# inferflow/inferflow

Hardware: AMD Instinct MI355X
Metric: decode tokens/sec, Llama-2-7B Q4 batch=1 greedy (whole job) (higher is better)
Workload: dtype i8 (Q8 activations x Q4_B32T1A weights, i32 dot, f32 scale, f16 I/O); 1 GPU; llama2_7b decode, Q4_B32T1A weights + F16 lm_head, F16 KV cache, batch 1 greedy, 16-token prompt, context 21..1851; parallelism=single, weights_bytes=4309647360

## Files before the change

inferflow_amd/csrc/ifa_decode_attn.h:

```cpp
#pragma once
#include "ifa_decode_kernels.h"
#include "ifa_decode_route.h"

namespace ifa {

struct DecAttnParams {
    const half_t *q;
    const half_t *k_new;
    const half_t *v_new;
    uint8_t *kcache, *vcache;
    const int *state;
    const float *rope_tab;
    int heads, kv_heads, kv_q8;
    float kq_scale;
    int rope_order, rope_cols;
    int alibi, alibi_base, alibi_total;
    half_t *out;
    int max_ctx;
    int8_t *xq;
    long long *trace;
    const void *batch_rows;
    int q_stride;
    int skip_store;
};
// ... 61 lines not shown
    int pos;
    unsigned *err;
    long long timeout_ticks;
    unsigned long long *att_gran;
};

__host__ __device__ inline int att_gran_count(int heads, int hd) { return heads * hd / 4 + 2 * (heads * hd / 32) + heads; }

template <int HD, bool Q8, int PB, bool KT>
struct DecAttnRegs {
    static constexpr int DG = HD / 8, NSPLIT = 256 / DG, VPRE = PB / NSPLIT;
    static constexpr int KBYTES = (HD / 32) * 34;
    static constexpr int KALIGN = HD == 128 ? 8 : (HD == 64 ? 4 : 2);
    uint32_t kreg[Q8 ? 1 : HD / 2];
    uint32_t kq32[(Q8 && KALIGN >= 4) ? KBYTES / 4 : 1];
    uint16_t kq16[(Q8 && KALIGN < 4) ? KBYTES / 2 : 1];
    u32x4 kt[KT ? PB / NSPLIT : 1];
    u32x4 vreg[Q8 ? 1 : VPRE];
    uint32_t vqs[Q8 ? VPRE : 1], vqc[Q8 ? VPRE : 1][2];
    float rope_cs, rope_sn;
    half_t q_in, k_in, v_in;
};

template <int HD, bool Q8, bool BATCH, int PB, bool KT, bool FUSED, int PHASE = 0>
__device__ __forceinline__ void dec_attn_body(char *smem, const half_t *pq, const uint8_t *pkc, const uint8_t *pvc, int pheads, int pkvh,
                                              const DecAttnParams &P, const int h_in, const DecAttnFusedIn &F, DecAttnRegs<HD, Q8, PB, KT> &R)
{
    int pos_b = 0;
    if constexpr (FUSED) pos_b = F.pos;
    if constexpr (BATCH) {
        const DecAttnBatchRow br = reinterpret_cast<const DecAttnBatchRow *>(P.batch_rows)[blockIdx.y];
        pkc = br.kc; pvc = br.vc; pos_b = br.n_ctx - 1;
        pq += (size_t)blockIdx.y * P.q_stride;
    }
#define IFA_GP(T, p) ((const __attribute__((address_space(1))) T *)(p))
    uint8_t *const kcw = BATCH ? const_cast<uint8_t *>(pkc) : P.kcache;
    uint8_t *const vcw = BATCH ? const_cast<uint8_t *>(pvc) : P.vcache;
    const float *const rope_tab = BATCH ? P.rope_tab + (size_t)blockIdx.y * HD : P.rope_tab;
    half_t *const outp = BATCH ? P.out + (size_t)blockIdx.y * pheads * HD : P.out;
    static_assert(HD % 8 == 0 && HD <= 128 && (!Q8 || HD % 32 == 0), "head size: multiples of 8 up to 128 (Q8 rows: whole 32-blocks)");
    constexpr int DG = HD / 8;
    constexpr int NSPLIT = 256 / DG;
    half_t *qs = reinterpret_cast<half_t *>(smem);
    half_t *kn = qs + HD;
    half_t *vn = kn + HD;
    float *red = reinterpret_cast<float *>(vn + HD);
    float *opart = red + 16;
    static_assert(!KT || (!Q8 && !BATCH && (DG & (DG - 1)) == 0 && PB % NSPLIT == 0), "K tile through LDS: F16 rows, one query, power-of-two pieces per row");
    static_assert(!(FUSED && BATCH), "the fused tail is a single-query kernel");
    static_assert(PB >= NSPLIT && PB <= DEC_ATTN_MIN_ROWS, "prefetch bucket");
    uint8_t *ktile = reinterpret_cast<uint8_t *>(opart + NSPLIT * HD);
    half_t *S = reinterpret_cast<half_t *>(ktile + (KT ? (size_t)PB * HD * 2 : 0));
    const int h = h_in, tid = threadIdx.x, lane = tid & 63, wave = tid >> 6;
    const int group = pheads / pkvh;
    const int kvh = h / group;
    bool writer = (h % group) == 0;
    if constexpr (BATCH) writer = writer && !P.skip_store;
    const int kv_dim = pkvh * HD;
    const size_t row_bytes = Q8 ? (size_t)(kv_dim / 32) * 34 : (size_t)kv_dim * 2;
    const size_t head_off = Q8 ? (size_t)((kvh * HD) / 32) * 34 : (size_t)kvh * HD * 2;

    constexpr int KBYTES = (HD / 32) * 34;
    constexpr int KALIGN = HD == 128 ? 8 : (HD == 64 ? 4 : 2);
    auto &kreg = R.kreg; auto &kq32 = R.kq32; auto &kq16 = R.kq16; auto &kt = R.kt; auto &vreg = R.vreg; auto &vqs = R.vqs; auto &vqc = R.vqc;
    float &rope_cs = R.rope_cs, &rope_sn = R.rope_sn;
    half_t &q_in = R.q_in, &k_in = R.k_in, &v_in = R.v_in;
    auto load_k = [&](int j) {
        const uint8_t *rowp = pkc + (size_t)j * row_bytes + head_off;
        if constexpr (Q8) {
            if constexpr (KALIGN == 8) {
#pragma unroll
                for (int i = 0; i < KBYTES / 8; i++) {
// ... 48 lines not shown
        const int j = min(sp + NSPLIT * i, BATCH ? pos_b : (FUSED ? min(pos_b, PB - 1) : PB - 1));
        if constexpr (!Q8) {
            vreg[i] = IFA_GP(u32x4, pvc + (size_t)j * row_bytes + head_off)[dg];
        } else {
            const auto *blk = IFA_GP(uint16_t, pvc + (size_t)j * row_bytes + vq_off);
            typedef uint32_t u32x2_a2 __attribute__((ext_vector_type(2), aligned(2)));
            vqs[i] = blk[0];
            const u32x2_a2 cw = *IFA_GP(u32x2_a2, blk + 1 + (dg % 4) * 4);
            vqc[i][0] = cw[0]; vqc[i][1] = cw[1];
        }
    }
    }
    if constexpr (PHASE == 1) return;

    const bool tr = P.trace != nullptr && tid == 0;
    if (tr) P.trace[h * 8 + 0] = wall_clock64();
    const int pos = (BATCH || FUSED) ? pos_b : *(const __attribute__((address_space(4))) int *)(P.state + 1);
    const int n_ctx = pos + 1;
    if constexpr (FUSED) {
        if (tid < HD) {
            const unsigned long long *gq = F.gran + (size_t)h * HD + tid, *gk = F.gran + (size_t)(pheads + kvh) * HD + tid,
                                     *gv = F.gran + (size_t)(pheads + pkvh + kvh) * HD + tid;
            const long long t_give_up = wall_clock64() + F.timeout_ticks;
            for (;;) {
                const unsigned long long a = __hip_atomic_load(gq, __ATOMIC_RELAXED, __HIP_MEMORY_SCOPE_AGENT);
                const unsigned long long b = __hip_atomic_load(gk, __ATOMIC_RELAXED, __HIP_MEMORY_SCOPE_AGENT);
                const unsigned long long c = __hip_atomic_load(gv, __ATOMIC_RELAXED, __HIP_MEMORY_SCOPE_AGENT);
                const bool ok = (unsigned)(a >> 32) == F.epoch && (unsigned)(b >> 32) == F.epoch && (unsigned)(c >> 32) == F.epoch;
                q_in = __builtin_bit_cast(half_t, (uint16_t)a); k_in = __builtin_bit_cast(half_t, (uint16_t)b); v_in = __builtin_bit_cast(half_t, (uint16_t)c);
                if (__all(ok)) break;
                if (wall_clock64() > t_give_up) { if (lane == 0) atomicExch(F.err, 0x51u); break; }
                __builtin_amdgcn_s_sleep(2);
            }
        }
    }
    if (tid < HD) { qs[tid] = q_in; kn[tid] = k_in; vn[tid] = v_in; }
    if constexpr (KT) {
#pragma unroll
        for (int i = 0; i < PB / NSPLIT; i++) {
            const int j = sp + NSPLIT * i;
            *reinterpret_cast<u32x4 *>(ktile + ((size_t)j * DG + (size_t)(dg ^ (j & (DG - 1)))) * 16) = kt[i];
        }
    }
    __syncthreads();
    if (tr) P.trace[h * 8 + 1] = wall_clock64();
    if (P.rope_order != 0) {
        if (tid < HD) {
            const int c = tid < HD / 2 ? tid : tid - HD / 2;
            rope_apply(tid < HD / 2 ? qs : kn, c, rope_cs, rope_sn, P.rope_order, P.rope_cols);
        }
        __syncthreads();
    }
    if constexpr (Q8) {
        constexpr int NB = HD / 32;
        for (int b = wave * 2 + (lane >> 5); b < 2 * NB; b += 8) {
            half_t *src = b < NB ? kn : vn;
            const int bb = b < NB ? b : b - NB;
            const int l32 = lane & 31;
            {
                const float val = h2f(src[bb * 32 + l32]);
                const float mx = half_wave_max(fabsf(val));
                const float sc = mx / 127;
                int qv = sc <= 0.000001f ? 0 : (int)roundf(val / sc);
                qv = min(max(qv, -128), 127);
                const half_t sch = f2h(sc);
                if (writer) {
                    uint8_t *cache = b < NB ? kcw : vcw;
                    uint8_t *blk = cache + (size_t)pos * row_bytes + head_off + (size_t)bb * 34;
                    blk[2 + l32] = (uint8_t)(int8_t)qv;
                    if (l32 == 0) *reinterpret_cast<uint16_t *>(blk) = __builtin_bit_cast(uint16_t, sch);
                }
                src[bb * 32 + l32] = f2h((float)qv * h2f(sch));
            }
        }
        __syncthreads();
    } else {
        if (writer && tid < HD) {
            reinterpret_cast<half_t *>(kcw + (size_t)pos * row_bytes + head_off)[tid] = kn[tid];
            reinterpret_cast<half_t *>(vcw + (size_t)pos * row_bytes + head_off)[tid] = vn[tid];
        }
    }

    if constexpr (KT) {
        if (tid < PB) {
#pragma unroll
            for (int i = 0; i < DG; i++) {
                const u32x4 t = *reinterpret_cast<const u32x4 *>(ktile + ((size_t)tid * DG + (size_t)(i ^ (tid & (DG - 1)))) * 16);
                kreg[4 * i] = t[0]; kreg[4 * i + 1] = t[1]; kreg[4 * i + 2] = t[2]; kreg[4 * i + 3] = t[3];
            }
        }
    }
    if (tr) P.trace[h * 8 + 2] = wall_clock64();
    const float alpha = 1.0f / sqrtf((float)HD) / P.kq_scale;
    const float mk = P.alibi ? alibi_slope(h + P.alibi_base, P.alibi_total) : 0.0f;
    float lmax = -INFINITY;
    uint32_t kreg2[(BATCH && !Q8) ? HD / 2 : 1];
    uint32_t kq32b[(BATCH && Q8 && KALIGN >= 4) ? KBYTES / 4 : 1];
    constexpr bool KPRE = BATCH && (!Q8 || KALIGN >= 4);
    bool have = false;
    for (int j = tid; j < n_ctx; j += 256) {
        ScoreAcc acc;
        if constexpr (KPRE) {
// ... 90 lines not shown
            const float inv0 = 1.0f / (((lsum0 + 0.0f) + 0.0f) + 0.0f);
            if (tid < n_ctx) S[tid] = f2h(h2f(f2h(e)) * inv0);
        }
        __syncthreads();
    } else {
    if (lane == 0) red[wave] = lmax;
    __syncthreads();
    if (tr) P.trace[h * 8 + 4] = wall_clock64();
    const float mx = fmaxf(fmaxf(red[0], red[1]), fmaxf(red[2], red[3]));
    float lsum = 0.0f;
    for (int j = tid; j < n_ctx; j += 256) {
        const float e = expf(P.kq_scale * h2f(S[j]) - mx);
        lsum += e;
        S[j] = f2h(e);
    }
    lsum = wave_sum(lsum);
    if (lane == 0) red[4 + wave] = lsum;
    __syncthreads();
    const float inv = 1.0f / (((red[4] + red[5]) + red[6]) + red[7]);
    for (int j = tid; j < n_ctx; j += 256) S[j] = f2h(h2f(S[j]) * inv);
    __syncthreads();
    }
    if (tr) P.trace[h * 8 + 5] = wall_clock64();

    float o[8];
#pragma unroll
    for (int i = 0; i < 8; i++) o[i] = 0.0f;
    auto acc_v = [&](float pj, const u32x4 vv) {
        const half8_t v8 = __builtin_bit_cast(half8_t, vv);
#pragma unroll
        for (int e = 0; e < 8; e++) o[e] = __builtin_fmaf(pj, (float)v8[e], o[e]);
    };
    auto acc_new = [&](float pj) {
#pragma unroll
        for (int e = 0; e < 8; e++) o[e] = __builtin_fmaf(pj, h2f(vn[dg * 8 + e]), o[e]);
    };
    auto acc_q8w = [&](float pj, uint16_t scb, uint16_t c0, uint16_t c1, uint16_t c2, uint16_t c3) {
        const half_t sch = __builtin_bit_cast(half_t, scb);
        const half2_t sc2 = {sch, sch};
        half2_t v01, v23, v45, v67;
        q8x4_dequant_h((uint32_t)c0 | ((uint32_t)c1 << 16), sc2, v01, v23);
        q8x4_dequant_h((uint32_t)c2 | ((uint32_t)c3 << 16), sc2, v45, v67);
        o[0] = __builtin_fmaf(pj, (float)v01[0], o[0]); o[1] = __builtin_fmaf(pj, (float)v01[1], o[1]);
        o[2] = __builtin_fmaf(pj, (float)v23[0], o[2]); o[3] = __builtin_fmaf(pj, (float)v23[1], o[3]);
        o[4] = __builtin_fmaf(pj, (float)v45[0], o[4]); o[5] = __builtin_fmaf(pj, (float)v45[1], o[5]);
        o[6] = __builtin_fmaf(pj, (float)v67[0], o[6]); o[7] = __builtin_fmaf(pj, (float)v67[1], o[7]);
    };
    auto acc_q8 = [&](float pj, int j) {
        const auto *blk = IFA_GP(uint16_t, pvc + (size_t)j * row_bytes + head_off + (size_t)(dg / 4) * 34);
        typedef uint32_t u32x2_a2 __attribute__((ext_vector_type(2), aligned(2)));
        const u32x2_a2 cw = *IFA_GP(u32x2_a2, blk + 1 + (dg % 4) * 4);
        acc_q8w(pj, blk[0], (uint16_t)(cw[0] & 0xFFFFu), (uint16_t)(cw[0] >> 16), (uint16_t)(cw[1] & 0xFFFFu), (uint16_t)(cw[1] >> 16));
    };
#pragma unroll
    for (int i = 0; i < VPRE; i++) {
        const int j = sp + NSPLIT * i;
        if (j < n_ctx && vact) {
            const float pj = h2f(S[j]);
            if (j == pos) acc_new(pj);
            else if constexpr (Q8) acc_q8w(pj, (uint16_t)vqs[i], (uint16_t)(vqc[i][0] & 0xFFFFu), (uint16_t)(vqc[i][0] >> 16), (uint16_t)(vqc[i][1] & 0xFFFFu), (uint16_t)(vqc[i][1] >> 16));
            else acc_v(pj, vreg[i]);
        }
    }
    {
        constexpr int TB = 8;
        u32x4 tcur[Q8 ? 1 : TB], tnxt[Q8 ? 1 : TB];
        uint32_t ts_c[Q8 ? TB : 1], tc_c[Q8 ? TB : 1][2], ts_n[Q8 ? TB : 1], tc_n[Q8 ? TB : 1][2];
        const size_t tq_off = head_off + (size_t)(dg / 4) * 34;
        auto tload = [&](u32x4 (&dst)[Q8 ? 1 : TB], uint32_t (&ds)[Q8 ? TB : 1], uint32_t (&dc)[Q8 ? TB : 1][2], int j) {
#pragma unroll
            for (int u = 0; u < TB; u++) {
                const int jr = min(j + u * NSPLIT, n_ctx - 1);
                if constexpr (!Q8) dst[u] = IFA_GP(u32x4, pvc + (size_t)jr * row_bytes + head_off)[dg];
                else {
                    const auto *blk = IFA_GP(uint16_t, pvc + (size_t)jr * row_bytes + tq_off);
                    typedef uint32_t u32x2_a2 __attribute__((ext_vector_type(2), aligned(2)));
                    ds[u] = blk[0];
                    const u32x2_a2 cw = *IFA_GP(u32x2_a2, blk + 1 + (dg % 4) * 4);
                    dc[u][0] = cw[0]; dc[u][1] = cw[1];
                }
            }
        };
        int j = vact ? sp + NSPLIT * VPRE : n_ctx;
        if (j < n_ctx) tload(tcur, ts_c, tc_c, j);
        for (; j < n_ctx; j += TB * NSPLIT) {
            tload(tnxt, ts_n, tc_n, j + TB * NSPLIT);
#pragma unroll
            for (int u = 0; u < TB; u++) {
                const int jj = j + u * NSPLIT;
                if (jj >= n_ctx) break;
                const float pj = h2f(S[jj]);
                if (jj == pos) acc_new(pj);
                else if constexpr (Q8) acc_q8w(pj, (uint16_t)ts_c[u], (uint16_t)(tc_c[u][0] & 0xFFFFu), (uint16_t)(tc_c[u][0] >> 16), (uint16_t)(tc_c[u][1] & 0xFFFFu), (uint16_t)(tc_c[u][1] >> 16));
                else acc_v(pj, tcur[u]);
            }
#pragma unroll
            for (int u = 0; u < TB; u++) {
                if constexpr (Q8) { ts_c[u] = ts_n[u]; tc_c[u][0] = tc_n[u][0]; tc_c[u][1] = tc_n[u][1]; }
                else tcur[u] = tnxt[u];
            }
        }
    }
    if (vact) {
#pragma unroll
        for (int e = 0; e < 8; e++) opart[sp * HD + dg * 8 + e] = o[e];
    }
    if (tr) P.trace[h * 8 + 6] = wall_clock64();
    __syncthreads();
    if (tid < HD) {
        float acc = opart[tid];
        for (int s2 = 1; s2 < NSPLIT; s2++) acc = acc + opart[s2 * HD + tid];
        const half_t yh = f2h(acc);
        outp[(size_t)h * HD + tid] = yh;
        if constexpr (HD % 32 == 0 && !BATCH) { if (P.xq) dec_attn_emit_q8<HD>(P.xq, P.heads * HD, h, tid, yh); }
        if constexpr (FUSED && HD % 32 == 0) {
            if (F.att_gran) {
                const float val = h2f(yh);
                const float mxv = half_wave_max(fabsf(val));
                const float qsc = mxv / 127;
                const int qv = q8_round_div1(val, qsc);
                const int sum = half_wave_sum_i32(qv);
                const int q1 = dpp_xor1(qv), q2 = dpp_xor2(qv), q3 = dpp_xor1(q2);
                const unsigned long long tagw = (unsigned long long)F.epoch << 32;
                const int cols = pheads * HD, nc = cols / 4, nbk = cols / 32;
                if ((tid & 3) == 0) {
                    const uint32_t w4 = (uint32_t)(qv & 0xFF) | ((uint32_t)(q1 & 0xFF) << 8) | ((uint32_t)(q2 & 0xFF) << 16) | ((uint32_t)(q3 & 0xFF) << 24);
                    __hip_atomic_store(F.att_gran + (h * HD + tid) / 4, tagw | w4, __ATOMIC_RELAXED, __HIP_MEMORY_SCOPE_AGENT);
                }
                if ((tid & 31) == 0) {
                    const int blk = (h * HD + tid) >> 5;
                    __hip_atomic_store(F.att_gran + nc + blk, tagw | __builtin_bit_cast(uint32_t, h2f(f2h(qsc))), __ATOMIC_RELAXED, __HIP_MEMORY_SCOPE_AGENT);
                    __hip_atomic_store(F.att_gran + nc + nbk + blk, tagw | __builtin_bit_cast(uint32_t, (float)sum), __ATOMIC_RELAXED, __HIP_MEMORY_SCOPE_AGENT);
                }
                if (tid == 0) __hip_atomic_store(F.att_gran + nc + 2 * nbk + h, tagw | 1u, __ATOMIC_RELAXED, __HIP_MEMORY_SCOPE_AGENT);
// ... 333 lines not shown
```

inferflow_amd/csrc/ifa_decode_kernels.h:

```cpp
#pragma once
#include "ifa_device.h"
#include "ifa_math.h"
#include "ifa_tiled.h"
#include "ifa_decode_formats.h"
#include "ifa_decode_gemv_plan.h"

namespace ifa {

typedef _Float16 half2_t __attribute__((ext_vector_type(2)));
typedef _Float16 half8_t __attribute__((ext_vector_type(8)));

__device__ __forceinline__ void q8_round_div8(const float (&v)[8], float qs, int (&q)[8])
{
    const float rqs = 1.0f / qs;
    bool risky = false;
#pragma unroll
    for (int i = 0; i < 8; i++) {
        const float t = v[i] * rqs;
        const float k = __builtin_rintf(t);
        risky |= fabsf(fabsf(t - k) - 0.5f) < 0.00006103515625f;
        q[i] = (int)k;
    }
    if (__builtin_expect(risky, 0)) {
#pragma unroll
// ... 47 lines not shown
    l.codes = reinterpret_cast<int8_t *>(smem); off += ((size_t)cols + 15) / 16 * 16;
    l.scale = reinterpret_cast<float *>(smem + off); off += nb * 4;
    l.xsum = reinterpret_cast<float *>(smem + off); off += nb * 4;
    off = (off + 15) / 16 * 16;
    l.part = reinterpret_cast<float *>(smem + off); off += 132 * 4;
    off = (off + 15) / 16 * 16;
    l.xh = reinterpret_cast<half_t *>(smem + off);
    return l;
}

struct XqImage {
    int8_t *codes; float *scale; float *xsum;
};
__host__ __device__ inline size_t xq_image_bytes(int cols) { return (((size_t)cols + 15) / 16 * 16) + ((size_t)cols / 32) * 8 + 16; }
__host__ __device__ inline XqImage xq_image_carve(void *base, int cols)
{
    XqImage q;
    q.codes = reinterpret_cast<int8_t *>(base);
    q.scale = reinterpret_cast<float *>(reinterpret_cast<char *>(base) + (((size_t)cols + 15) / 16 * 16));
    q.xsum = q.scale + cols / 32;
    return q;
}

__device__ __forceinline__ void lds_counter_add(float *slot)
{
    asm volatile("" ::: "memory");
    __hip_atomic_fetch_add(reinterpret_cast<uint32_t *>(slot), 1u, __ATOMIC_RELAXED, __HIP_MEMORY_SCOPE_WORKGROUP);
}
__device__ __forceinline__ void lds_counter_wait(float *slot, uint32_t target)
{
    volatile uint32_t *c = reinterpret_cast<volatile uint32_t *>(slot);
    while (__builtin_amdgcn_readfirstlane(*c) < target) __builtin_amdgcn_s_sleep(1);
    asm volatile("" ::: "memory");
}

template <int NORM, int MAXC, bool XADD = false, int NT = 0>
struct XPre {
    static __device__ __forceinline__ int nthr() { return NT ? NT : (int)blockDim.x; }
    half8_t xv[MAXC];
    half8_t wv[NORM ? MAXC : 1], bv[NORM ? MAXC : 1];
    half8_t av[XADD ? MAXC : 1], abv[XADD ? MAXC : 1];

    __device__ __forceinline__ void issue_add(const half_t *__restrict__ add, const half_t *__restrict__ add_bias, int cols)
    {
        const int chunks = cols >> 3;
#pragma unroll
        for (int k = 0; k < MAXC; k++) {
            const int c = threadIdx.x + k * (int)blockDim.x;
            if (c < chunks) {
                av[k] = *reinterpret_cast<const half8_t *>(add + (size_t)c * 8);
                if (add_bias) abv[k] = *reinterpret_cast<const half8_t *>(add_bias + (size_t)c * 8);
            }
        }
    }
// ... 738 lines not shown
```

inferflow_amd/csrc/ifa_decode_qkv_attn.h:

```cpp
#pragma once
#include "ifa_decode_kernels.h"
#include "ifa_decode_attn.h"

namespace ifa {

struct DecQkvAttnExtra {
    unsigned long long *gran;
    const unsigned *epoch;
    unsigned epoch_add;
    unsigned *err;
    int timeout_us;
    int gk;
    int unload;
};

#ifndef IFA_QA_EARLY_KV
#define IFA_QA_EARLY_KV 0
#endif
#ifndef IFA_QA_WARM_ROWS
#define IFA_QA_WARM_ROWS 1
#endif
constexpr int QA_THREADS = 512;

template <int DT, int NJ, int RW, int NORM, int HD, bool Q8, int PB, bool KT, int NP, bool UL = false>
__global__ void __launch_bounds__(QA_THREADS) k_dec_qkv_attn(const half_t *px, const half_t *pnw, const half_t *pnb, int pcols, int pgeo,
                                                             const uint8_t *pwq, const uint8_t *pwk, const uint8_t *pwv,
                                                             const DecGemvParams P, const DecAttnParams A, const DecQkvAttnExtra E)
{
    const int g_heads = pgeo & 0xFF, g_kvh = (pgeo >> 8) & 0xFF, g_gk = (pgeo >> 16) & 0xFFFF;
    const int g_nblk = pcols / block_capacity(DT);
    extern __shared__ __attribute__((aligned(16))) char smem[];
    const long long t_kernel = wall_clock64();
    static_assert(NORM == 0 || NORM == 1, "QKV prologue: quantiser with or without the RMS norm");
    static_assert(NP > 0 && NP * 64 < QA_THREADS, "wave-specialised prologue");
    constexpr int TH = QA_THREADS, PT = NP * 64;
    constexpr int MAXC = (NJ * 8 * block_capacity(DT) + PT - 1) / PT;
    XPre<NORM, MAXC, false, PT> pre;
    if (threadIdx.x < PT) pre.issue(px, pnw, pnb, pcols);
    const XLds L = xlds_carve(smem, pcols);
    const int lane = threadIdx.x & 63;
    const int wave = __builtin_amdgcn_readfirstlane(threadIdx.x >> 6);
    using Fmt = DecFmt<DT, NJ>;
    const size_t row_bytes = tiled_row_bytes(DT, (size_t)g_nblk);
    const int g = (int)blockIdx.x / g_gk, bg = (int)blockIdx.x - g * g_gk;
    const int group = g_heads / g_kvh;
    const int RG = (group + 2) * HD;
    const int per = g_gk / group;
    const bool attn_wg = bg % per == 0;
    const int head = g * group + bg / per;
    const int WGV = UL ? (g_gk - group) * (TH / 64) : g_gk * (TH / 64);
    const int lw = UL ? (bg - bg / per - 1) * (TH / 64) + wave : bg * (TH / 64) + wave;
    struct Row { const uint8_t *w; const half_t *b; half_t *y; int row, vrow; };
    auto locate = [&](int lr) {
        Row r;
        const int nq = group * HD;
        const bool isk = lr >= nq && lr < nq + HD, isv = lr >= nq + HD;
        r.row = isv ? g * HD + (lr - nq - HD) : (isk ? g * HD + (lr - nq) : g * nq + lr);
        r.w = isv ? P.W0[2] : (isk ? P.W0[1] : P.W0[0]);
        r.b = isv ? P.b0[2] : (isk ? P.b0[1] : P.b0[0]);
        r.y = isv ? P.y[2] : (isk ? P.y[1] : P.y[0]);
        r.vrow = isv ? (g_heads + g_kvh) * HD + r.row : (isk ? g_heads * HD + r.row : r.row);
        return r;
    };
    typename Fmt::W w[RW];
    auto wrow = [&](int lr) -> const uint8_t * {
        const int nq = group * HD;
        const bool isk = lr >= nq && lr < nq + HD, isv = lr >= nq + HD;
        const int row = isv ? g * HD + (lr - nq - HD) : (isk ? g * HD + (lr - nq) : g * nq + lr);
        const uint64_t q = (uint64_t)pwq, dk = (uint64_t)pwk - q, dv = (uint64_t)pwv - q;
        return (const uint8_t *)(q + (isk ? dk : 0) + (isv ? dv : 0)) + (size_t)row * row_bytes;
    };
    auto load_rows = [&](int i0, int i1) {
        const bool full = (RW - 1) * WGV + lw < RG;
        if (full) {
#pragma unroll
            for (int i = 0; i < RW; i++) { if (i < i0 || i >= i1) continue; w[i].load(wrow(i * WGV + lw), g_nblk, lane); }
        } else {
#pragma unroll
            for (int i = 0; i < RW; i++) {
                if (i < i0 || i >= i1) continue;
                if (i > 0 && i * WGV + lw >= RG) continue;
                w[i].load(wrow(min(i * WGV + lw, RG - 1)), g_nblk, lane);
            }
        }
    };
    static_assert(NP == 4, "the prologue waves are the attention waves");
    const bool ul_head = UL && attn_wg;
    if (!ul_head && threadIdx.x == TH - 1) { L.part[130] = 0.0f; L.part[131] = 0.0f; }
    if (!ul_head && wave >= NP) load_rows(0, 1);
    const int pos = *(const __attribute__((address_space(4))) int *)(A.state + 1);
    const unsigned epoch = ((*(const __attribute__((address_space(4))) unsigned *)(E.epoch) + E.epoch_add) << 20) | ((unsigned)pos & 0xFFFFFu);
    DecAttnFusedIn F;
    F.gran = E.gran; F.epoch = epoch; F.pos = pos; F.err = E.err; F.timeout_ticks = (long long)E.timeout_us * 100;
    F.att_gran = nullptr;
    if constexpr (UL) {
        if (attn_wg) {
            if (wave >= 4) {
#if IFA_QA_WARM_ROWS
                if (pos >= PB) {
                    constexpr int SB = Q8 ? (HD / 32) * 34 : HD * 2;
                    const int kvh = head / group, kv_dim = g_kvh * HD;
                    const size_t rb = Q8 ? (size_t)(kv_dim / 32) * 34 : (size_t)kv_dim * 2;
                    const size_t ho = Q8 ? (size_t)((kvh * HD) / 32) * 34 : (size_t)kvh * HD * 2;
                    const int t = (int)threadIdx.x - 256;
                    const int off = min((t & 3) * 64, SB - 4) & ~1;
                    typedef uint32_t u32_a2 __attribute__((aligned(2)));
                    uint32_t acc = 0;
                    for (int j = PB + (t >> 2); j <= pos; j += 64) {
                        acc ^= *(const __attribute__((address_space(1))) u32_a2 *)(A.kcache + (size_t)j * rb + ho + off);
                        acc ^= *(const __attribute__((address_space(1))) u32_a2 *)(A.vcache + (size_t)j * rb + ho + off);
                    }
                    if (acc == 0x9E3779B9u && A.trace) A.trace[(size_t)A.heads * 8 + 7] = (long long)acc;
                }
#endif
                return;
            }
            DecAttnRegs<HD, Q8, PB, KT> RU;
            dec_attn_body<HD, Q8, false, PB, KT, true>(smem, nullptr, A.kcache, A.vcache, A.heads, A.kv_heads, A, head, F, RU);
            return;
        }
    }
    __syncthreads();
    DecAttnRegs<HD, Q8, PB, KT> R;
    if (wave >= NP) {
        load_rows(1, RW);
    } else {
        pre.finish(P.norm_w, P.norm_b, P.multi_base, P.eps, P.cols, L, P.xn_out, nullptr);
        load_rows(0, RW);
#if IFA_QA_EARLY_KV
        if (attn_wg) dec_attn_body<HD, Q8, false, PB, KT, true, 1>(smem, nullptr, A.kcache, A.vcache, A.heads, A.kv_heads, A, head, F, R);
#endif
    }
    lds_counter_wait(L.part + 131, NP);
    typename Fmt::X X;
    X.load(L.codes, L.scale, L.xsum, lane, g_nblk);
    {
        float a[RW];
#pragma unroll
        for (int i = 0; i < RW; i++) a[i] = w[i].dot(X);
#pragma unroll
        for (int i = 0; i < RW; i++) a[i] = wave_sum(a[i]);
        float a0 = 0.0f;
#pragma unroll
        for (int i = 0; i < RW; i++) { if (lane == i) a0 = a[i]; }
        const int lr = lane * WGV + lw;
        if (lane < RW && lr < RG) {
            const Row r = locate(lr);
            half_t y = dec_bias(a0, r.b, r.row);
            if (P.pre_scale != 0.0f) y = f2h(h2f(y) * P.pre_scale);
            r.y[r.row] = y;
            __hip_atomic_store(E.gran + r.vrow, ((unsigned long long)epoch << 32) | (unsigned long long)__builtin_bit_cast(uint16_t, y),
                               __ATOMIC_RELAXED, __HIP_MEMORY_SCOPE_AGENT);
        }
    }
    if (A.trace && threadIdx.x == 0) {
        A.trace[(size_t)(A.heads + (int)blockIdx.x) * 8 + 0] = t_kernel;
        A.trace[(size_t)(A.heads + (int)blockIdx.x) * 8 + 1] = wall_clock64();
    }
    if (attn_wg) {
        __syncthreads();
        if (wave >= 4) return;
        dec_attn_body<HD, Q8, false, PB, KT, true, IFA_QA_EARLY_KV ? 2 : 0>(smem, nullptr, A.kcache, A.vcache, A.heads, A.kv_heads, A, head, F, R);
        return;
    }
}

bool dec_qkv_attn_supported(int w_dtype, int cols, int heads, int kv_heads, int head_dim, int num_cus, int *gk_out, int *rw_out);
int dec_qkv_attn_launch(int w_dtype, int norm, bool kv_q8, int pb, bool kt, bool ul, const DecGemvParams &P, const DecAttnParams &A, const DecQkvAttnExtra &E,
                        int max_ctx, hipStream_t s);
template <int DT>
int dec_qkv_attn_launch_dt(int norm, bool kv_q8, int pb, bool kt, bool ul, int rw, const DecGemvParams &P, const DecAttnParams &A, const DecQkvAttnExtra &E,
                           int max_ctx, hipStream_t s);

}
```

inferflow_amd/csrc/ifa_engine.hip:

```cpp
#include <mutex>
#include <unordered_map>
#include "ifa_engine_state.h"

namespace ifa {

namespace {
struct SpaceBook {
    std::mutex mu;
    std::unordered_map<void *, size_t> live;
    long long live_bytes = 0, fail_at = 0;
};
SpaceBook &book() { static SpaceBook *b = new SpaceBook(); return *b; }

template <class Alloc> int space_alloc(const char *call, void **p, size_t bytes, Alloc alloc)
{
    SpaceBook &b = book();
    *p = nullptr;
    {
        std::lock_guard<std::mutex> g(b.mu);
        if (b.fail_at > 0 && --b.fail_at == 0)
            return ifa_fail(IFA_ERR_HIP, "%s(%zu bytes) failed: out of memory (simulated: ifa_debug_alloc_fail_at)", call, bytes);
    }
    const hipError_t e = alloc(p, bytes);
    if (e != hipSuccess) {
// ... 475 lines not shown
    if (slot == m->cur_slot) return IFA_OK;
    if (m->tp_graph_exec) { (void)hipGraphExecDestroy(m->tp_graph_exec); m->tp_graph_exec = nullptr; }
    if (m->tp_graph) { (void)hipGraphDestroy(m->tp_graph); m->tp_graph = nullptr; }
    ifa_model::KvSlot &out = m->slots[(size_t)m->cur_slot], &in = m->slots[(size_t)slot];
    out.k.clear(); out.v.clear();
    for (Layer &L : m->layers) { out.k.push_back(std::move(L.kcache)); out.v.push_back(std::move(L.vcache)); }
    out.graph = m->graph; out.exec = m->graph_exec;
    if (m->graph_exec_n) { (void)hipGraphExecDestroy(m->graph_exec_n); m->graph_exec_n = nullptr; }
    if (m->graph_n) { (void)hipGraphDestroy(m->graph_n); m->graph_n = nullptr; }
    for (size_t l = 0; l < m->layers.size(); l++) { m->layers[l].kcache = std::move(in.k[l]); m->layers[l].vcache = std::move(in.v[l]); }
    m->graph = in.graph; m->graph_exec = in.exec;
    in.k.clear(); in.v.clear(); in.graph = nullptr; in.exec = nullptr;
    m->cur_slot = slot;
    return IFA_OK;
}

int ifa_model_set_option(ifa_model *m, const char *name, int value)
{
    IFA_REQUIRE(m && name, "ifa_model_set_option: null pointer");
    if (strcmp(name, "pool_lse") == 0) { m->opt_pool_lse = value != 0; return IFA_OK; }
    struct { const char *n; int *p; } opts[] = {
        {"fused", &m->opt_fused}, {"graph", &m->opt_graph}, {"rpw_qkv", &m->opt_rpw_qkv}, {"rpw_wo", &m->opt_rpw_wo},
        {"rpw_ffn", &m->opt_rpw_ffn}, {"rpw_w2", &m->opt_rpw_w2}, {"rpw_lm", &m->opt_rpw_lm}, {"trace", &m->opt_trace},
        {"bench_mode", &m->opt_bench_mode}, {"touch_stride", &m->opt_touch_stride}, {"attn_split_ctx", &m->opt_attn_split_ctx}, {"batch_graph", &m->opt_batch_graph}, {"gemm_rows", &m->opt_gemm_rows}, {"batch_fused", &m->opt_batch_fused}, {"rows_mo", &m->opt_rows_mo}, {"debug_mo_alloc_fail", &m->opt_debug_mo_alloc_fail}, {"rows_kparts", &m->opt_rows_kparts}, {"prefill_chunk", &m->opt_prefill_chunk}, {"prefill_big_min", &m->opt_prefill_big_min}, {"prefill_mid", &m->opt_prefill_mid}, {"prefill_mid_max", &m->opt_prefill_mid_max}, {"prefill_res_mid", &m->opt_prefill_res_mid}, {"gemm_splitk", &m->opt_gemm_splitk}, {"moe_singles", &m->opt_moe_singles}, {"moe_overlap", &m->opt_moe_overlap}, {"prefill_big", &m->opt_prefill_big}, {"moe_router_fused", &m->opt_moe_router_fused}, {"tp_fuse_add", &m->opt_tp_fuse_add}, {"attn_q8", &m->opt_attn_q8}, {"attn_kt", &m->opt_attn_kt}, {"fuse_attn", &m->opt_fuse_attn}, {"fuse_ffn", &m->opt_fuse_ffn}, {"attn_post_as_residual", &m->opt_attn_post_as_residual}, {"chain_late_w2", &m->opt_chain_late_w2}, {"exact_order", &m->opt_exact_order}, {"perf_stat", &m->opt_perf_stat}, {"attn_nsplits", &m->opt_attn_nsplits}, {"attn_unload", &m->opt_attn_unload}, {"q3h_native", &m->opt_q3h_native}, {"fuse_attn_timeout_us", &m->opt_fuse_attn_timeout_us}, {"step_tail", &m->opt_step_tail}, {"graph_steps", &m->opt_graph_steps}, {"moe_device", &m->opt_moe_device}, 
        
        {"debug_layers", &m->opt_debug_layers}, {"debug_layer0", &m->opt_debug_layer0}, {"debug_hidden_in", &m->opt_debug_hidden_in}};
    for (auto &o : opts)
        if (strcmp(o.n, name) == 0) {
            *o.p = value;
            drop_graphs(m);
            return IFA_OK;
        }
    return ifa_fail(IFA_ERR_ARG, "ifa_model_set_option: unknown option '%s'", name);
}

int ifa_model_perf_stat(ifa_model *m, int *keys_out, float *ms_out, int cap, int *n_out, int clear)
{
    IFA_REQUIRE(m && n_out && cap >= 0 && (cap == 0 || (keys_out && ms_out)), "ifa_model_perf_stat: null pointer");
    IFA_HIP_CHECK(hipSetDevice(m->cfg.device));
    int rc = perf_collect(m);
    if (rc) return rc;
    int n = 0;
    for (auto &kv : m->perf_map) {
        if (n < cap) { keys_out[n] = kv.first; ms_out[n] = kv.second; }
        n++;
    }
    *n_out = n;
// ... 145 lines not shown
```

inferflow_amd/csrc/ifa_engine_decode.hip:

```cpp
#include "ifa_engine_state.h"

namespace ifae {


__global__ void __launch_bounds__(256) k_touch(const uint8_t *__restrict__ p, size_t bytes, size_t stride, int *sink)
{
    size_t i = ((size_t)blockIdx.x * blockDim.x + threadIdx.x) * stride;
    int acc = 0;
    for (; i < bytes; i += (size_t)gridDim.x * blockDim.x * stride) acc += *reinterpret_cast<const int *>(p + i);
    if (acc == 0x7FFFFFFF) *sink = acc;
}

static long long *g_trace_ptr = nullptr;

bool fused_ok(const Tensor &t, bool long_rows)
{
    if (!t.present()) return false;
    if (fused_int8(t.dtype)) return t.tiled && (long_rows ? dec_gemv_supported_long(t.dtype, t.cols) : dec_gemv_supported(t.dtype, t.cols));
    return dec_gemv_h_supported(t.dtype, t.cols) && (long_rows || t.cols <= 8192);
}

template <int EPI, int NORM>
static int launch_dec_gemv(int w_dtype, const DecGemvParams &P, int wgs_per_cu_opt, hipStream_t s)
{
// ... 805 lines not shown
        return rc;
    }
    if (elapsed_ms) { IFA_HIP_CHECK(hipEventElapsedTime(elapsed_ms, e0, e1)); (void)hipEventDestroy(e0); (void)hipEventDestroy(e1); }
    if (out_tokens_host) memcpy(out_tokens_host, m->host_pinned + 8, sizeof(int) * (size_t)n_steps);
    th("done");
    return IFA_OK;
}

}

extern "C" {

int ifa_model_time_kernel(ifa_model *m, int which, int iters, float *avg_us)
{
    IFA_REQUIRE(m && m->finalized && avg_us, "ifa_model_time_kernel: bad arguments");
    IFA_REQUIRE(iters > 0 && which >= 0 && which <= 9, "ifa_model_time_kernel: which %d iters %d", which, iters);
    IFA_HIP_CHECK(hipSetDevice(m->cfg.device));
    std::string why;
    if (!fused_supported(m, &why)) return ifa_fail(IFA_ERR_STATE, "fused path unavailable: %s", why.c_str());
    int rc = ensure_scratch(m, 1);
    if (rc) return rc;
    if (m->opt_q3h_native && (rc = ensure_q3hn(m))) return rc;
    hipStream_t s = m->stream;
    m->host_pinned[0] = 1; m->host_pinned[1] = std::min(m->cfg.max_ctx - 1, 64); m->host_pinned[2] = 0;
    IFA_HIP_CHECK(hipMemcpyAsync(m->state, m->host_pinned, 3 * sizeof(int), hipMemcpyHostToDevice, s));
    auto touch_layer = [&](int l) {
        const int ids[] = {T_WQ, T_WK, T_WV, T_WO, T_W1, T_W3, T_W2};
        for (int id : ids) {
            const Tensor &t = m->layers[(size_t)l].t[id];
            if (!t.tiled) continue;
            const size_t bytes = t.rows * ifa_tiled_row_bytes(t.dtype, t.cols);
            k_touch<<<dim3(8), dim3(256), 0, s>>>((const uint8_t *)t.tiled, bytes, (size_t)m->opt_touch_stride, m->state + 7);
        }
    };
    if ((rc = decode_route_ready(m, m->route_reach))) return rc;
    if (which == 9 && !m->route.chain) return ifa_fail(IFA_ERR_STATE, "chained FFN launch unavailable for this model / option set");
    if (which == 7 && m->route.kind != DEC_ROUTE_FUSED_TAIL) return ifa_fail(IFA_ERR_STATE, "fused QKV + attention launch unavailable for this model / option set");
    auto one = [&](int i) -> int {
        if (which == 7) return launch_qkv_attn(m, i % m->cfg.layers, m->x, (unsigned)(i + 1));
        if (which == 9) return launch_chain(m, i % m->cfg.layers, m->x, m->x2, (unsigned)(i + 1));
        const int l = m->opt_bench_mode == 1 ? 0 : i % m->cfg.layers;
        if (m->opt_bench_mode == 2) touch_layer(l);
        switch (which) {
        case 0: return launch_qkv(m, l, m->x);
        case 1: return launch_attn(m, l);
        case 2: return launch_wo(m, l, m->x);
        case 3: return launch_ffn13(m, l, -1, m->x);
// ... 27 lines not shown
```

inferflow_amd/csrc/ifa_engine_state.h:

```cpp
#pragma once
#include <chrono>
#include <cstdlib>
#include <cstring>
#include <map>
#include <string>
#include <type_traits>
#include <vector>
#include "ifa_host.h"
#include "ifa_buf_hip.h"
#include "ifa_decode_kernels.h"
#include "ifa_decode_attn.h"
#include "ifa_decode_gemv.h"
#include "ifa_moe.h"
#include "ifa_gemm_rows_mfma.h"
#include "ifa_gemm_big.h"
#include "ifa_decode_lmhead_tail.h"
#include "ifa_decode_singles.h"
#include "ifa_decode_qkv_attn.h"
#include "ifa_decode_chain.h"
#include "ifa_prompt_route.h"

using namespace ifa;

namespace ifae {
// ... 43 lines not shown
    DevBuf<uint8_t> moe_xq_in, moe_xq_mid;
    DevBuf<void> moe_tiles, moe_singles, moe_smalls;
    DevBuf<int> tokens_dev;
    DevBuf<half_t> pn;
};


}
using namespace ifae;

struct ifa_model : Scratch {
    ifa_model_config cfg;
    std::vector<Layer> layers;
    Tensor g[10];
    hipStream_t stream = nullptr;
    hipStream_t side_stream = nullptr; Event ev_fork, ev_join; int opt_moe_overlap = 1;
    bool own_stream = true;
    bool finalized = false;
    int opt_moe_device = 1;
    DevBuf<int> state;
    DevBuf<float> rope_tab;
    DevBuf<long long> trace;
    int opt_trace = 0, opt_bench_mode = 0, opt_touch_stride = 65536;
    PinBuf<int> host_pinned;
    int scratch_tokens = 0;
    size_t kv_row_bytes = 0;
    hipGraph_t graph = nullptr;
    hipGraphExec_t graph_exec = nullptr;
    hipGraph_t graph_n = nullptr; hipGraphExec_t graph_exec_n = nullptr; int graph_n_steps = 0, opt_graph_steps = 1;
    struct PendingAdd { const half_t *x = nullptr, *add = nullptr, *bias = nullptr; half_t *out = nullptr; bool on = false; } pend;
    int opt_tp_fuse_add = 1;
    DevPin<void> batch_tab;
    std::map<int, hipGraphExec_t> batch_graphs;
    std::map<int, hipGraphExec_t> draft_graphs;
    DecAttnSplitWs attn_ws = {nullptr, nullptr, nullptr, 8};
    DevBuf<half_t> attn_ws_S; DevBuf<float> attn_ws_lmax, attn_ws_opart;
    int opt_attn_unload = 1;
    int opt_attn_nsplits = 0;
    DecRoute route; int route_reach = 256;
    PromptRoute prompt_route;
    int opt_fuse_attn = 1, opt_fuse_attn_timeout_us = 20000;
    DevBuf<unsigned long long> qa_gran;
    DevBuf<unsigned> qa_call, qa_err; unsigned qa_calls = 0;
    int opt_fuse_ffn = 0, opt_chain_late_w2 = 0;
    int opt_q3h_native = 0;
    int opt_perf_stat = 0;
// ... 251 lines not shown
```

Baseline: 627.1 tokens/s.

## Stage fused QKV+attention so attention waits only on Q/K before V

Adds a compile-time staged mode where the fused attention tail waits only for Q and K granules, computes scores and the cached-V accumulation, and only then waits for the new V row. The new token's V is quantised, stored, and folded into the split partial sums at the end. The QKV producer is meant to emit Q/K rows in an earlier stage so attention can start sooner. Staging is off by default (IFA_QA_STAGED=0). Unconditionally active are a simplified row-load path with precomputed bias/output pointers, LDS address-space casts on the counters, and a bench option for the timed position.

New measurement: 635.6 tokens/s (median of 6 runs). +1.4%, better.

```diff
diff --git a/inferflow_amd/csrc/ifa_decode_attn.h b/inferflow_amd/csrc/ifa_decode_attn.h
--- a/inferflow_amd/csrc/ifa_decode_attn.h
+++ b/inferflow_amd/csrc/ifa_decode_attn.h
@@ -107,7 +107,7 @@
     half_t q_in, k_in, v_in;
 };
 
-template <int HD, bool Q8, bool BATCH, int PB, bool KT, bool FUSED, int PHASE = 0>
+template <int HD, bool Q8, bool BATCH, int PB, bool KT, bool FUSED, int PHASE = 0, bool STG = false>
 __device__ __forceinline__ void dec_attn_body(char *smem, const half_t *pq, const uint8_t *pkc, const uint8_t *pvc, int pheads, int pkvh,
                                               const DecAttnParams &P, const int h_in, const DecAttnFusedIn &F, DecAttnRegs<HD, Q8, PB, KT> &R)
 {
@@ -133,6 +133,7 @@
     float *opart = red + 16;
     static_assert(!KT || (!Q8 && !BATCH && (DG & (DG - 1)) == 0 && PB % NSPLIT == 0), "K tile through LDS: F16 rows, one query, power-of-two pieces per row");
     static_assert(!(FUSED && BATCH), "the fused tail is a single-query kernel");
+    static_assert(!STG || (FUSED && PHASE == 0), "the two waits are the fused tail's");
     static_assert(PB >= NSPLIT && PB <= DEC_ATTN_MIN_ROWS, "prefetch bucket");
     uint8_t *ktile = reinterpret_cast<uint8_t *>(opart + NSPLIT * HD);
     half_t *S = reinterpret_cast<half_t *>(ktile + (KT ? (size_t)PB * HD * 2 : 0));
@@ -227,6 +228,17 @@
             const unsigned long long *gq = F.gran + (size_t)h * HD + tid, *gk = F.gran + (size_t)(pheads + kvh) * HD + tid,
                                      *gv = F.gran + (size_t)(pheads + pkvh + kvh) * HD + tid;
             const long long t_give_up = wall_clock64() + F.timeout_ticks;
+            if constexpr (STG) {
+                for (;;) {
+                    const unsigned long long a = __hip_atomic_load(gq, __ATOMIC_RELAXED, __HIP_MEMORY_SCOPE_AGENT);
+                    const unsigned long long b = __hip_atomic_load(gk, __ATOMIC_RELAXED, __HIP_MEMORY_SCOPE_AGENT);
+                    const bool ok = (unsigned)(a >> 32) == F.epoch && (unsigned)(b >> 32) == F.epoch;
+                    q_in = __builtin_bit_cast(half_t, (uint16_t)a); k_in = __builtin_bit_cast(half_t, (uint16_t)b);
+                    if (__all(ok)) break;
+                    if (wall_clock64() > t_give_up) { if (lane == 0) atomicExch(F.err, 0x51u); break; }
+                    __builtin_amdgcn_s_sleep(2);
+                }
+            } else
             for (;;) {
                 const unsigned long long a = __hip_atomic_load(gq, __ATOMIC_RELAXED, __HIP_MEMORY_SCOPE_AGENT);
                 const unsigned long long b = __hip_atomic_load(gk, __ATOMIC_RELAXED, __HIP_MEMORY_SCOPE_AGENT);
@@ -258,7 +270,7 @@
     }
     if constexpr (Q8) {
         constexpr int NB = HD / 32;
-        for (int b = wave * 2 + (lane >> 5); b < 2 * NB; b += 8) {
+        for (int b = wave * 2 + (lane >> 5); b < (STG ? NB : 2 * NB); b += 8) {
             half_t *src = b < NB ? kn : vn;
             const int bb = b < NB ? b : b - NB;
             const int l32 = lane & 31;
@@ -282,7 +294,7 @@
     } else {
         if (writer && tid < HD) {
             reinterpret_cast<half_t *>(kcw + (size_t)pos * row_bytes + head_off)[tid] = kn[tid];
-            reinterpret_cast<half_t *>(vcw + (size_t)pos * row_bytes + head_off)[tid] = vn[tid];
+            if constexpr (!STG) reinterpret_cast<half_t *>(vcw + (size_t)pos * row_bytes + head_off)[tid] = vn[tid];
         }
     }
 
@@ -419,6 +431,10 @@
     __syncthreads();
     }
     if (tr) P.trace[h * 8 + 5] = wall_clock64();
+
+    unsigned long long v_look = 0;
+    if constexpr (STG)
+        v_look = __hip_atomic_load(F.gran + (size_t)(pheads + pkvh + kvh) * HD + dq, __ATOMIC_RELAXED, __HIP_MEMORY_SCOPE_AGENT);
 
     float o[8];
 #pragma unroll
@@ -454,7 +470,7 @@
         const int j = sp + NSPLIT * i;
         if (j < n_ctx && vact) {
             const float pj = h2f(S[j]);
-            if (j == pos) acc_new(pj);
+            if (j == pos) { if constexpr (!STG) acc_new(pj); }
             else if constexpr (Q8) acc_q8w(pj, (uint16_t)vqs[i], (uint16_t)(vqc[i][0] & 0xFFFFu), (uint16_t)(vqc[i][0] >> 16), (uint16_t)(vqc[i][1] & 0xFFFFu), (uint16_t)(vqc[i][1] >> 16));
             else acc_v(pj, vreg[i]);
         }
@@ -487,7 +503,7 @@
                 const int jj = j + u * NSPLIT;
                 if (jj >= n_ctx) break;
                 const float pj = h2f(S[jj]);
-                if (jj == pos) acc_new(pj);
+                if (jj == pos) { if constexpr (!STG) acc_new(pj); }
                 else if constexpr (Q8) acc_q8w(pj, (uint16_t)ts_c[u], (uint16_t)(tc_c[u][0] & 0xFFFFu), (uint16_t)(tc_c[u][0] >> 16), (uint16_t)(tc_c[u][1] & 0xFFFFu), (uint16_t)(tc_c[u][1] >> 16));
                 else acc_v(pj, tcur[u]);
             }
@@ -505,8 +521,52 @@
     if (tr) P.trace[h * 8 + 6] = wall_clock64();
     __syncthreads();
     if (tid < HD) {
-        float acc = opart[tid];
-        for (int s2 = 1; s2 < NSPLIT; s2++) acc = acc + opart[s2 * HD + tid];
+        float acc;
+        if constexpr (STG) {
+            {
+                const unsigned long long *gv = F.gran + (size_t)(pheads + pkvh + kvh) * HD + tid;
+                const long long t_give_up = wall_clock64() + F.timeout_ticks;
+                for (;;) {
+                    const bool ok = (unsigned)(v_look >> 32) == F.epoch;
+                    v_in = __builtin_bit_cast(half_t, (uint16_t)v_look);
+                    if (__all(ok)) break;
+                    if (wall_clock64() > t_give_up) { if (lane == 0) atomicExch(F.err, 0x52u); break; }
+                    __builtin_amdgcn_s_sleep(2);
+                    v_look = __hip_atomic_load(gv, __ATOMIC_RELAXED, __HIP_MEMORY_SCOPE_AGENT);
+                }
+            }
+            if (tr) P.trace[(size_t)(pheads + (int)blockIdx.x) * 8 + 5] = wall_clock64();
+            half_t vv = v_in;
+            if constexpr (Q8) {
+                const int bb = tid >> 5, l32 = lane & 31;
+                const float val = h2f(vv);
+                const float mx = half_wave_max(fabsf(val));
+                const float sc = mx / 127;
+                int qv = sc <= 0.000001f ? 0 : (int)roundf(val / sc);
+                qv = min(max(qv, -128), 127);
+                const half_t sch = f2h(sc);
+                if (writer) {
+                    uint8_t *blk = vcw + (size_t)pos * row_bytes + head_off + (size_t)bb * 34;
+                    blk[2 + l32] = (uint8_t)(int8_t)qv;
+                    if (l32 == 0) *reinterpret_cast<uint16_t *>(blk) = __builtin_bit_cast(uint16_t, sch);
+                }
+                vv = f2h((float)qv * h2f(sch));
+            } else {
+                if (writer) reinterpret_cast<half_t *>(vcw + (size_t)pos * row_bytes + head_off)[tid] = vv;
+            }
+            const int sp_new = pos % NSPLIT;
+            const float p_new = h2f(S[pos]), v_new = h2f(vv);
+            acc = opart[tid];
+            if (sp_new == 0) acc = __builtin_fmaf(p_new, v_new, acc);
+            for (int s2 = 1; s2 < NSPLIT; s2++) {
+                float part = opart[s2 * HD + tid];
+                if (s2 == sp_new) part = __builtin_fmaf(p_new, v_new, part);
+                acc = acc + part;
+            }
+        } else {
+            acc = opart[tid];
+            for (int s2 = 1; s2 < NSPLIT; s2++) acc = acc + opart[s2 * HD + tid];
+        }
         const half_t yh = f2h(acc);
         outp[(size_t)h * HD + tid] = yh;
         if constexpr (HD % 32 == 0 && !BATCH) { if (P.xq) dec_attn_emit_q8<HD>(P.xq, P.heads * HD, h, tid, yh); }
diff --git a/inferflow_amd/csrc/ifa_decode_kernels.h b/inferflow_amd/csrc/ifa_decode_kernels.h
--- a/inferflow_amd/csrc/ifa_decode_kernels.h
+++ b/inferflow_amd/csrc/ifa_decode_kernels.h
@@ -93,14 +93,15 @@
     return q;
 }
 
+typedef __attribute__((address_space(3))) uint32_t lds_u32;
 __device__ __forceinline__ void lds_counter_add(float *slot)
 {
     asm volatile("" ::: "memory");
-    __hip_atomic_fetch_add(reinterpret_cast<uint32_t *>(slot), 1u, __ATOMIC_RELAXED, __HIP_MEMORY_SCOPE_WORKGROUP);
+    __hip_atomic_fetch_add((lds_u32 *)reinterpret_cast<uint32_t *>(slot), 1u, __ATOMIC_RELAXED, __HIP_MEMORY_SCOPE_WORKGROUP);
 }
 __device__ __forceinline__ void lds_counter_wait(float *slot, uint32_t target)
 {
-    volatile uint32_t *c = reinterpret_cast<volatile uint32_t *>(slot);
+    volatile lds_u32 *c = (volatile lds_u32 *)reinterpret_cast<uint32_t *>(slot);
     while (__builtin_amdgcn_readfirstlane(*c) < target) __builtin_amdgcn_s_sleep(1);
     asm volatile("" ::: "memory");
 }
diff --git a/inferflow_amd/csrc/ifa_decode_qkv_attn.h b/inferflow_amd/csrc/ifa_decode_qkv_attn.h
--- a/inferflow_amd/csrc/ifa_decode_qkv_attn.h
+++ b/inferflow_amd/csrc/ifa_decode_qkv_attn.h
@@ -20,7 +20,17 @@
 #ifndef IFA_QA_WARM_ROWS
 #define IFA_QA_WARM_ROWS 1
 #endif
+#ifndef IFA_QA_STAGED
+#define IFA_QA_STAGED 0
+#endif
 constexpr int QA_THREADS = 512;
+
+template <int N, typename F>
+__device__ __forceinline__ void qa_stage_dispatch(int s, F &&f)
+{
+    if constexpr (N <= 1) f(std::integral_constant<int, 1>{});
+    else { if (s >= N) f(std::integral_constant<int, N>{}); else qa_stage_dispatch<N - 1>(s, f); }
+}
 
 template <int DT, int NJ, int RW, int NORM, int HD, bool Q8, int PB, bool KT, int NP, bool UL = false>
 __global__ void __launch_bounds__(QA_THREADS) k_dec_qkv_attn(const half_t *px, const half_t *pnw, const half_t *pnb, int pcols, int pgeo,
@@ -50,15 +60,18 @@
     const int head = g * group + bg / per;
     const int WGV = UL ? (g_gk - group) * (TH / 64) : g_gk * (TH / 64);
     const int lw = UL ? (bg - bg / per - 1) * (TH / 64) + wave : bg * (TH / 64) + wave;
-    struct Row { const uint8_t *w; const half_t *b; half_t *y; int row, vrow; };
+    typedef __attribute__((address_space(1))) half_t g_half;
+    struct Row { const g_half *b; g_half *y; int row, vrow; bool has_b; };
+    uint64_t pb_q = 0, pb_k = 0, pb_v = 0, py_q = 0, py_k = 0, py_v = 0;
     auto locate = [&](int lr) {
         Row r;
         const int nq = group * HD;
         const bool isk = lr >= nq && lr < nq + HD, isv = lr >= nq + HD;
         r.row = isv ? g * HD + (lr - nq - HD) : (isk ? g * HD + (lr - nq) : g * nq + lr);
-        r.w = isv ? P.W0[2] : (isk ? P.W0[1] : P.W0[0]);
-        r.b = isv ? P.b0[2] : (isk ? P.b0[1] : P.b0[0]);
-        r.y = isv ? P.y[2] : (isk ? P.y[1] : P.y[0]);
+        const uint64_t b = pb_q + (isk ? pb_k - pb_q : 0) + (isv ? pb_v - pb_q : 0);
+        r.has_b = b != 0;
+        r.b = (const g_half *)b;
+        r.y = (g_half *)(py_q + (isk ? py_k - py_q : 0) + (isv ? py_v - py_q : 0));
         r.vrow = isv ? (g_heads + g_kvh) * HD + r.row : (isk ? g_heads * HD + r.row : r.row);
         return r;
     };
@@ -71,25 +84,20 @@
         return (const uint8_t *)(q + (isk ? dk : 0) + (isv ? dv : 0)) + (size_t)row * row_bytes;
     };
     auto load_rows = [&](int i0, int i1) {
-        const bool full = (RW - 1) * WGV + lw < RG;
-        if (full) {
-#pragma unroll
-            for (int i = 0; i < RW; i++) { if (i < i0 || i >= i1) continue; w[i].load(wrow(i * WGV + lw), g_nblk, lane); }
-        } else {
-#pragma unroll
-            for (int i = 0; i < RW; i++) {
-                if (i < i0 || i >= i1) continue;
-                if (i > 0 && i * WGV + lw >= RG) continue;
-                w[i].load(wrow(min(i * WGV + lw, RG - 1)), g_nblk, lane);
-            }
+#pragma unroll
+        for (int i = 0; i < RW; i++) {
+            if (i < i0 || i >= i1) continue;
+            const int lr = i * WGV + lw;
+            w[i].load(wrow(lr < RG ? lr : min(lw, RG - 1)), g_nblk, lane);
         }
     };
     static_assert(NP == 4, "the prologue waves are the attention waves");
     const bool ul_head = UL && attn_wg;
     if (!ul_head && threadIdx.x == TH - 1) { L.part[130] = 0.0f; L.part[131] = 0.0f; }
-    if (!ul_head && wave >= NP) load_rows(0, 1);
     const int pos = *(const __attribute__((address_space(4))) int *)(A.state + 1);
     const unsigned epoch = ((*(const __attribute__((address_space(4))) unsigned *)(E.epoch) + E.epoch_add) << 20) | ((unsigned)pos & 0xFFFFFu);
+    pb_q = (uint64_t)P.b0[0]; pb_k = (uint64_t)P.b0[1]; pb_v = (uint64_t)P.b0[2];
+    py_q = (uint64_t)P.y[0]; py_k = (uint64_t)P.y[1]; py_v = (uint64_t)P.y[2];
     DecAttnFusedIn F;
     F.gran = E.gran; F.epoch = epoch; F.pos = pos; F.err = E.err; F.timeout_ticks = (long long)E.timeout_us * 100;
     F.att_gran = nullptr;
@@ -116,17 +124,15 @@
                 return;
             }
             DecAttnRegs<HD, Q8, PB, KT> RU;
-            dec_attn_body<HD, Q8, false, PB, KT, true>(smem, nullptr, A.kcache, A.vcache, A.heads, A.kv_heads, A, head, F, RU);
+            dec_attn_body<HD, Q8, false, PB, KT, true, 0, (IFA_QA_STAGED != 0)>(smem, nullptr, A.kcache, A.vcache, A.heads, A.kv_heads, A, head, F, RU);
             return;
         }
     }
     __syncthreads();
     DecAttnRegs<HD, Q8, PB, KT> R;
-    if (wave >= NP) {
-        load_rows(1, RW);
-    } else {
-        pre.finish(P.norm_w, P.norm_b, P.multi_base, P.eps, P.cols, L, P.xn_out, nullptr);
-        load_rows(0, RW);
+    if (wave < NP) pre.finish(P.norm_w, P.norm_b, P.multi_base, P.eps, P.cols, L, P.xn_out, nullptr);
+    load_rows(0, RW);
+    if (wave < NP) {
 #if IFA_QA_EARLY_KV
         if (attn_wg) dec_attn_body<HD, Q8, false, PB, KT, true, 1>(smem, nullptr, A.kcache, A.vcache, A.heads, A.kv_heads, A, head, F, R);
 #endif
@@ -137,20 +143,40 @@
     {
         float a[RW];
 #pragma unroll
-        for (int i = 0; i < RW; i++) a[i] = w[i].dot(X);
-#pragma unroll
-        for (int i = 0; i < RW; i++) a[i] = wave_sum(a[i]);
-        float a0 = 0.0f;
-#pragma unroll
-        for (int i = 0; i < RW; i++) { if (lane == i) a0 = a[i]; }
-        const int lr = lane * WGV + lw;
-        if (lane < RW && lr < RG) {
-            const Row r = locate(lr);
-            half_t y = dec_bias(a0, r.b, r.row);
-            if (P.pre_scale != 0.0f) y = f2h(h2f(y) * P.pre_scale);
-            r.y[r.row] = y;
-            __hip_atomic_store(E.gran + r.vrow, ((unsigned long long)epoch << 32) | (unsigned long long)__builtin_bit_cast(uint16_t, y),
-                               __ATOMIC_RELAXED, __HIP_MEMORY_SCOPE_AGENT);
+        for (int i = 0; i < RW; i++) a[i] = 0.0f;
+        auto stage = [&](auto lo_c, auto hi_c) {
+            constexpr int LO = decltype(lo_c)::value, HI = decltype(hi_c)::value;
+            if constexpr (LO < HI) {
+#pragma unroll
+                for (int i = LO; i < HI; i++) a[i] = w[i].dot(X);
+#pragma unroll
+                for (int i = LO; i < HI; i++) a[i] = wave_sum(a[i]);
+                const bool mine = lane >= LO && lane < HI && lane * WGV + lw < RG;
+                float a0 = a[0];
+#pragma unroll
+                for (int i = (LO > 1 ? LO : 1); i < HI; i++) { if (lane == i) a0 = a[i]; }
+                const Row r = locate(mine ? lane * WGV + lw : min(lw, RG - 1));
+                half_t y = f2h(a0);
+                if (r.has_b) y = f2h(h2f(y) + h2f(r.b[r.row]));
+                if (P.pre_scale != 0.0f) y = f2h(h2f(y) * P.pre_scale);
+                r.y[r.row] = y;
+                __hip_atomic_store(E.gran + r.vrow, ((unsigned long long)epoch << 32) | (unsigned long long)__builtin_bit_cast(uint16_t, y),
+                                   __ATOMIC_RELAXED, __HIP_MEMORY_SCOPE_AGENT);
+            }
+        };
+        auto staged = [&](auto s1_c) {
+            constexpr int S1 = decltype(s1_c)::value;
+            stage(std::integral_constant<int, 0>{}, s1_c);
+            if constexpr (S1 < RW) {
+                if (A.trace && threadIdx.x == 0) A.trace[(size_t)(A.heads + (int)blockIdx.x) * 8 + 2] = wall_clock64();
+            }
+            stage(s1_c, std::integral_constant<int, RW>{});
+        };
+        if constexpr (IFA_QA_STAGED != 0 && UL) {
+            const int s1 = min(RW, ((group + 1) * HD + WGV - 1) / WGV);
+            qa_stage_dispatch<RW>(s1, staged);
+        } else {
+            staged(std::integral_constant<int, RW>{});
         }
     }
     if (A.trace && threadIdx.x == 0) {
diff --git a/inferflow_amd/csrc/ifa_engine.hip b/inferflow_amd/csrc/ifa_engine.hip
--- a/inferflow_amd/csrc/ifa_engine.hip
+++ b/inferflow_amd/csrc/ifa_engine.hip
@@ -521,7 +521,7 @@
     struct { const char *n; int *p; } opts[] = {
         {"fused", &m->opt_fused}, {"graph", &m->opt_graph}, {"rpw_qkv", &m->opt_rpw_qkv}, {"rpw_wo", &m->opt_rpw_wo},
         {"rpw_ffn", &m->opt_rpw_ffn}, {"rpw_w2", &m->opt_rpw_w2}, {"rpw_lm", &m->opt_rpw_lm}, {"trace", &m->opt_trace},
-        {"bench_mode", &m->opt_bench_mode}, {"touch_stride", &m->opt_touch_stride}, {"attn_split_ctx", &m->opt_attn_split_ctx}, {"batch_graph", &m->opt_batch_graph}, {"gemm_rows", &m->opt_gemm_rows}, {"batch_fused", &m->opt_batch_fused}, {"rows_mo", &m->opt_rows_mo}, {"debug_mo_alloc_fail", &m->opt_debug_mo_alloc_fail}, {"rows_kparts", &m->opt_rows_kparts}, {"prefill_chunk", &m->opt_prefill_chunk}, {"prefill_big_min", &m->opt_prefill_big_min}, {"prefill_mid", &m->opt_prefill_mid}, {"prefill_mid_max", &m->opt_prefill_mid_max}, {"prefill_res_mid", &m->opt_prefill_res_mid}, {"gemm_splitk", &m->opt_gemm_splitk}, {"moe_singles", &m->opt_moe_singles}, {"moe_overlap", &m->opt_moe_overlap}, {"prefill_big", &m->opt_prefill_big}, {"moe_router_fused", &m->opt_moe_router_fused}, {"tp_fuse_add", &m->opt_tp_fuse_add}, {"attn_q8", &m->opt_attn_q8}, {"attn_kt", &m->opt_attn_kt}, {"fuse_attn", &m->opt_fuse_attn}, {"fuse_ffn", &m->opt_fuse_ffn}, {"attn_post_as_residual", &m->opt_attn_post_as_residual}, {"chain_late_w2", &m->opt_chain_late_w2}, {"exact_order", &m->opt_exact_order}, {"perf_stat", &m->opt_perf_stat}, {"attn_nsplits", &m->opt_attn_nsplits}, {"attn_unload", &m->opt_attn_unload}, {"q3h_native", &m->opt_q3h_native}, {"fuse_attn_timeout_us", &m->opt_fuse_attn_timeout_us}, {"step_tail", &m->opt_step_tail}, {"graph_steps", &m->opt_graph_steps}, {"moe_device", &m->opt_moe_device}, 
+        {"bench_mode", &m->opt_bench_mode}, {"touch_stride", &m->opt_touch_stride}, {"time_pos", &m->opt_time_pos}, {"attn_split_ctx", &m->opt_attn_split_ctx}, {"batch_graph", &m->opt_batch_graph}, {"gemm_rows", &m->opt_gemm_rows}, {"batch_fused", &m->opt_batch_fused}, {"rows_mo", &m->opt_rows_mo}, {"debug_mo_alloc_fail", &m->opt_debug_mo_alloc_fail}, {"rows_kparts", &m->opt_rows_kparts}, {"prefill_chunk", &m->opt_prefill_chunk}, {"prefill_big_min", &m->opt_prefill_big_min}, {"prefill_mid", &m->opt_prefill_mid}, {"prefill_mid_max", &m->opt_prefill_mid_max}, {"prefill_res_mid", &m->opt_prefill_res_mid}, {"gemm_splitk", &m->opt_gemm_splitk}, {"moe_singles", &m->opt_moe_singles}, {"moe_overlap", &m->opt_moe_overlap}, {"prefill_big", &m->opt_prefill_big}, {"moe_router_fused", &m->opt_moe_router_fused}, {"tp_fuse_add", &m->opt_tp_fuse_add}, {"attn_q8", &m->opt_attn_q8}, {"attn_kt", &m->opt_attn_kt}, {"fuse_attn", &m->opt_fuse_attn}, {"fuse_ffn", &m->opt_fuse_ffn}, {"attn_post_as_residual", &m->opt_attn_post_as_residual}, {"chain_late_w2", &m->opt_chain_late_w2}, {"exact_order", &m->opt_exact_order}, {"perf_stat", &m->opt_perf_stat}, {"attn_nsplits", &m->opt_attn_nsplits}, {"attn_unload", &m->opt_attn_unload}, {"q3h_native", &m->opt_q3h_native}, {"fuse_attn_timeout_us", &m->opt_fuse_attn_timeout_us}, {"step_tail", &m->opt_step_tail}, {"graph_steps", &m->opt_graph_steps}, {"moe_device", &m->opt_moe_device}, 
         
         {"debug_layers", &m->opt_debug_layers}, {"debug_layer0", &m->opt_debug_layer0}, {"debug_hidden_in", &m->opt_debug_hidden_in}};
     for (auto &o : opts)
diff --git a/inferflow_amd/csrc/ifa_engine_decode.hip b/inferflow_amd/csrc/ifa_engine_decode.hip
--- a/inferflow_amd/csrc/ifa_engine_decode.hip
+++ b/inferflow_amd/csrc/ifa_engine_decode.hip
@@ -851,7 +851,7 @@
     if (rc) return rc;
     if (m->opt_q3h_native && (rc = ensure_q3hn(m))) return rc;
     hipStream_t s = m->stream;
-    m->host_pinned[0] = 1; m->host_pinned[1] = std::min(m->cfg.max_ctx - 1, 64); m->host_pinned[2] = 0;
+    m->host_pinned[0] = 1; m->host_pinned[1] = std::min(m->cfg.max_ctx - 1, m->opt_time_pos >= 0 ? m->opt_time_pos : 64); m->host_pinned[2] = 0;
     IFA_HIP_CHECK(hipMemcpyAsync(m->state, m->host_pinned, 3 * sizeof(int), hipMemcpyHostToDevice, s));
     auto touch_layer = [&](int l) {
         const int ids[] = {T_WQ, T_WK, T_WV, T_WO, T_W1, T_W3, T_W2};
diff --git a/inferflow_amd/csrc/ifa_engine_state.h b/inferflow_amd/csrc/ifa_engine_state.h
--- a/inferflow_amd/csrc/ifa_engine_state.h
+++ b/inferflow_amd/csrc/ifa_engine_state.h
@@ -89,6 +89,7 @@
     DevBuf<float> rope_tab;
     DevBuf<long long> trace;
     int opt_trace = 0, opt_bench_mode = 0, opt_touch_stride = 65536;
+    int opt_time_pos = -1;
     PinBuf<int> host_pinned;
     int scratch_tokens = 0;
     size_t kv_row_bytes = 0;
```
